# GStreamer/gst-plugins-rs

Measured on AMD Instinct MI355X. Metric: 4K RGBA frames/sec through hsvfilter+colorlut at 1 GPU; % HBM roofline, higher is better.
Workload: dtype u8

## Files before the change

gst-plugins-rs_amd/csrc/group.hip:

```cpp
#include "internal.hpp"

#include <chrono>
#include <condition_variable>
#include <algorithm>
#include <cstring>
#include <deque>
#include <mutex>
#include <unordered_map>
#include <vector>

using namespace mi355;

namespace {

struct Desc {
  mi355_ctx *ctx;
  uint8_t *src, *dst;
  int width, height, stride, format;
  mi355_hsv_settings hs;
  const uint32_t *table;
  std::shared_ptr<void> table_ref;
  bool batchable;
  bool fused;
  uint64_t ticket;
  hipEvent_t ready;
};

struct Batch {
  uint64_t seq;
  std::vector<uint64_t> tickets;
  hipEvent_t done;
  int waiters;
  std::shared_ptr<void> table_ref;
};

struct GroupCore {
  int device = 0;
  std::mutex mu;
  std::vector<hipEvent_t> events;
  uint64_t next_ticket = 1;
  std::string last_error;
};

hipEvent_t take_event(GroupCore *g) {
  if (!g->events.empty()) { hipEvent_t e = g->events.back(); g->events.pop_back(); return e; }
  hipEvent_t e = nullptr;
  if (hipEventCreateWithFlags(&e, hipEventDisableTiming) != hipSuccess) { (void)hipGetLastError(); return nullptr; }
  return e;
}

int fail(GroupCore *g, int status, const std::string &msg) {
  g->last_error = msg;
  return status;
}

int record_ready(GroupCore *g, mi355_ctx *ctx, hipEvent_t *ready) {
  *ready = nullptr;
  if (hipStreamQuery(ctx->stream) == hipSuccess) return MI355_OK;
  (void)hipGetLastError();
  hipEvent_t e = take_event(g);
  if (!e || hipEventRecord(e, ctx->stream) != hipSuccess) {
    (void)hipGetLastError();
    if (e) g->events.push_back(e);
    return fail(g, MI355_ERR_HIP, "group: hipEventRecord(ready)");
  }
  *ready = e;
  return MI355_OK;
}

enum class Waited { kNothing , kDone, kFailed };
template <class S>
Waited wait_seq_unlocking(std::deque<S> &sets, uint64_t seq, std::unique_lock<std::mutex> &lk) {
  S *mine = nullptr;
  for (S &s : sets)
    if (s.seq == seq) { mine = &s; break; }
  if (!mine) return Waited::kNothing;
  const hipEvent_t ev = mine->done;
  mine->waiters++;
  lk.unlock();
  const hipError_t e = hipEventSynchronize(ev);
  lk.lock();
  for (S &s : sets)
    if (s.seq == seq) { s.waiters--; break; }
  if (e != hipSuccess) { (void)hipGetLastError(); return Waited::kFailed; }
  return Waited::kDone;
}

// ... 622 lines not shown
        const auto deadline = std::chrono::steady_clock::now() + std::chrono::microseconds(linger_us);
        while (is_pending(ticket) && (int)pending.size() < expected) {
          if (cv.wait_until(lk, deadline) == std::cv_status::timeout) break;
        }
      }
      if (is_pending(ticket)) (void)flush_locked(g, ticket);
    }
    if (int rc = wait_unlocking(g, lk, ticket)) return rc;
    auto r = results.find(ticket);
    if (r == results.end()) return fail(g, MI355_ERR_INVALID_ARG, std::string("group: this ") + Kind::kItem + "'s result has been collected already");
    *out = std::move(r->second);
    results.erase(r);
    if (const int status = Kind::status(*out)) return fail(g, status, std::string("group: the launch that carried this ") + Kind::kItem + " failed");
    return MI355_OK;
  }

  void stats(uint64_t out[4]) const {
    out[0] = n_items;
    out[1] = n_sets;
    out[2] = n_largest;
    out[3] = n_launches;
  }

  void destroy(GroupCore *g) {
    if (!kind.lane_stream(0)) return;
    if (kind.set_up()) {
      std::lock_guard<std::mutex> lk(g->mu);
      (void)flush_locked(g);
    }
    for (int l = 0; l < kind.lanes(); l++) (void)hipStreamSynchronize(kind.lane_stream(l));
    for (Set &s : sets) {
      (void)hipEventDestroy(s.done);
      kind.blocks.give(&s.data.block);
    }
    sets.clear();
    for (Item &d : pending)
      if (d.ready) (void)hipEventDestroy(d.ready);
    pending.clear();
    kind.destroy();
  }
};

}

struct mi355_group : GroupCore {
  int max_batch = 8;
  hipStream_t stream = nullptr;
  std::vector<Desc> pending;
  std::deque<Batch> batches;
  std::unordered_map<uint64_t, uint64_t> where;
  std::unordered_map<uint64_t, int> failed;
  uint64_t next_seq = 1;
  uint64_t n_frames = 0, n_batched_launch_pairs = 0, n_single = 0;
  std::vector<std::shared_ptr<void>> dead_refs;
  SetQueue<CmpKind> cmp;
  SetQueue<CdKind> cd;
  SetQueue<HdKind> hd;
  SetQueue<YdKind> yd;
  SetQueue<HnKind> hn;
  SetQueue<HfKind> hf;
};

namespace {

struct Locked {
  std::vector<std::shared_ptr<void>> reap;
  mi355_group *g;
  std::unique_lock<std::mutex> lk;
  explicit Locked(mi355_group *g_) : g(g_), lk(g_->mu) {}
  ~Locked() {
    if (!lk.owns_lock()) lk.lock();
    reap.swap(g->dead_refs);
    lk.unlock();
  }
};

void retire_front(mi355_group *g) {
  Batch &b = g->batches.front();
  for (uint64_t t : b.tickets) g->where.erase(t);
  g->events.push_back(b.done);
  if (b.table_ref) g->dead_refs.push_back(std::move(b.table_ref));
  g->batches.pop_front();
}

void retire_done(mi355_group *g) {
  while (!g->batches.empty() && g->batches.front().waiters == 0) {
    if (hipEventQuery(g->batches.front().done) != hipSuccess) { (void)hipGetLastError(); break; }
    retire_front(g);
  }
}

bool same_class(const Desc &a, const Desc &b) {
  return a.batchable && b.batchable && a.fused == b.fused && a.width == b.width && a.height == b.height && a.stride == b.stride && a.format == b.format && a.table == b.table &&
         std::memcmp(&a.hs, &b.hs, sizeof(a.hs)) == 0 && a.ctx->force_generic == b.ctx->force_generic;
}

int flush_locked(mi355_group *g, uint64_t until = 0) {
  bool reached = false;
  while (!g->pending.empty() && !reached) {
    std::vector<Desc> take, keep;
    std::vector<mi355_ctx *> blocked;
    const Desc first = g->pending.front();
    for (const Desc &d : g->pending) {
      bool stream_blocked = false;
      for (mi355_ctx *c : blocked) stream_blocked |= c == d.ctx;
      const bool fits = take.empty() || (!stream_blocked && (int)take.size() < g->max_batch && same_class(first, d));
      if (fits) take.push_back(d);
      else keep.push_back(d);
      if (!stream_blocked) blocked.push_back(d.ctx);
    }
    g->pending.swap(keep);
    PixFmt fmt;
    (void)pixfmt_of(first.format, &fmt);
    hipEvent_t done = take_event(g);
    if (!done) return fail(g, MI355_ERR_HIP, "hipEventCreate");
    int rc = MI355_OK;
    if (first.batchable) {
      uint8_t *srcs[kMultiFrames], *dsts[kMultiFrames];
      for (size_t i = 0; i < take.size(); i++) {
        srcs[i] = take[i].src;
        dsts[i] = take[i].dst;
        if (take[i].ready && hipStreamWaitEvent(g->stream, take[i].ready, 0) != hipSuccess) rc = MI355_ERR_HIP;
      }
      if (!rc && !first.fused) rc = launch_hsvfilter_multi(first.ctx, g->stream, srcs, (int)take.size(), first.width, first.height, fmt, first.hs);
      if (!rc) rc = launch_colorlut_multi(first.ctx, g->stream, first.table, srcs, dsts, (int)take.size(), first.width, first.height, first.fused);
      if (!rc && hipEventRecord(done, g->stream) != hipSuccess) rc = MI355_ERR_HIP;
      g->n_batched_launch_pairs++;
    } else {
      const Desc &d = take[0];
      const size_t pitch = (size_t)d.stride * (size_t)d.height;
      if (!g->batches.empty() && hipStreamWaitEvent(d.ctx->stream, g->batches.back().done, 0) != hipSuccess) rc = MI355_ERR_HIP;
      if (!rc && d.fused) rc = launch_hsv_colorlut(d.ctx, d.src, pitch, d.stride, d.dst, pitch, d.stride, 1, d.width, d.height, d.hs);
      if (!rc && !d.fused) rc = launch_hsvfilter(d.ctx, d.src, 1, pitch, d.width, d.height, d.stride, fmt, d.hs);
      if (!rc && !d.fused) rc = launch_colorlut(d.ctx, d.src, pitch, d.stride, d.dst, pitch, d.stride, 1, d.width, d.height, d.format);
      if (!rc && hipEventRecord(done, d.ctx->stream) != hipSuccess) rc = MI355_ERR_HIP;
      if (!rc && hipStreamWaitEvent(g->stream, done, 0) != hipSuccess) rc = MI355_ERR_HIP;
      if (rc && rc != MI355_ERR_HIP) g->last_error = d.ctx->last_error;
      g->n_single++;
    }
    for (const Desc &d : take)
      if (d.ready) g->events.push_back(d.ready);
    if (rc) {
      (void)hipGetLastError();
      g->events.push_back(done);
      if (g->failed.size() > 65536) g->failed.clear();
      for (const Desc &d : take) g->failed[d.ticket] = rc;
      if (g->last_error.empty()) g->last_error = "group launch failed";
      return rc;
    }
    Batch b{g->next_seq++, {}, done, 0, first.batchable ? first.table_ref : std::shared_ptr<void>()};
    for (const Desc &d : take) { b.tickets.push_back(d.ticket); g->where[d.ticket] = b.seq; reached |= until != 0 && d.ticket == until; }
    g->batches.push_back(std::move(b));
    g->n_frames += take.size();
  }
  return MI355_OK;
}

int wait_unlocking(mi355_group *g, std::unique_lock<std::mutex> &lk, uint64_t ticket) {
  auto bad = g->failed.find(ticket);
  if (bad != g->failed.end()) {
    const int rc = bad->second;
    g->failed.erase(bad);
    return fail(g, rc, "group: the launch that carried this frame failed");
  }
  auto it = g->where.find(ticket);
  if (it == g->where.end()) return MI355_OK;
  const uint64_t seq = it->second;
  const Waited w = wait_seq_unlocking(g->batches, seq, lk);
  if (w == Waited::kNothing) return MI355_OK;
  if (w == Waited::kFailed) return fail(g, MI355_ERR_HIP, "hipEventSynchronize(group batch)");
  while (!g->batches.empty() && g->batches.front().seq <= seq && g->batches.front().waiters == 0) retire_front(g);
  return MI355_OK;
}

int wait_all_unlocking(mi355_group *g, std::unique_lock<std::mutex> &lk) {
  while (!g->batches.empty()) {
    const uint64_t t = g->batches.back().tickets.back();
    const size_t before = g->batches.size();
    int rc = wait_unlocking(g, lk, t);
    if (rc) return rc;
    if (!g->batches.empty() && g->batches.size() >= before && g->batches.back().tickets.back() == t) break;
  }
  return MI355_OK;
}


template <class F>
void for_each_queue_but_compare(mi355_group *g, F &&f) {
  f(g->cd);
  f(g->hd);
  f(g->yd);
  f(g->hn);
  f(g->hf);
}

template <class F>
void for_each_set_queue(mi355_group *g, F &&f) {
  f(g->cmp);
  for_each_queue_but_compare(g, f);
}

int refuse_set_queue_ticket(mi355_group *g, uint64_t ticket) {
  std::string owner;
  for_each_queue_but_compare(g, [&](auto &q) {
    if (owner.empty() && q.owns(ticket)) owner = q.foreign_refusal();
  });
  return owner.empty() ? MI355_OK : fail(g, MI355_ERR_INVALID_ARG, owner);
}


template <class Q>
int queue_set_rendezvous(mi355_group *g, Q mi355_group::*q, int expected_streams, unsigned linger_us) {
  if (!g || expected_streams < 0) return MI355_ERR_INVALID_ARG;
  Locked L(g);
  (g->*q).set_rendezvous(expected_streams, linger_us);
  return MI355_OK;
}

template <class Q>
int queue_stats(mi355_group *g, Q mi355_group::*q, uint64_t *stats, int columns = 4) {
  if (!g || !stats) return MI355_ERR_INVALID_ARG;
  std::lock_guard<std::mutex> lk(g->mu);
  uint64_t all[4];
  (g->*q).stats(all);
  std::copy(all, all + columns, stats);
  return MI355_OK;
}

template <class Q>
int queue_wait_status(mi355_group *g, Q mi355_group::*q, uint64_t ticket) {
  if (!g) return MI355_ERR_INVALID_ARG;
  Locked L(g);
  int status = MI355_OK;
  return (g->*q).wait(g, L.lk, ticket, &status);
}

}

extern "C" {

mi355_group *mi355_group_create(int device, int max_batch, int *status) {
  if (max_batch < 0 || max_batch > kMultiFrames) { if (status) *status = MI355_ERR_INVALID_ARG; return nullptr; }
  if (hipSetDevice(device) != hipSuccess) { (void)hipGetLastError(); if (status) *status = MI355_ERR_NO_DEVICE; return nullptr; }
  mi355_group *g = new mi355_group();
  g->device = device;
  g->max_batch = max_batch ? max_batch : 8;
  if (hipStreamCreateWithFlags(&g->stream, hipStreamNonBlocking) != hipSuccess) {
    (void)hipGetLastError();
    delete g;
    if (status) *status = MI355_ERR_HIP;
    return nullptr;
  }
  if (status) *status = MI355_OK;
  return g;
}

void mi355_group_destroy(mi355_group *g) {
  if (!g) return;
  (void)hipSetDevice(g->device);
  {
    Locked L(g);
    (void)flush_locked(g);
    (void)wait_all_unlocking(g, L.lk);
  }
  (void)hipStreamSynchronize(g->stream);
  for_each_set_queue(g, [&](auto &q) { q.destroy(g); });
  for (Batch &b : g->batches) (void)hipEventDestroy(b.done);
  for (Desc &d : g->pending)
    if (d.ready) (void)hipEventDestroy(d.ready);
  g->pending.clear();
  g->batches.clear();
  g->dead_refs.clear();
  for (hipEvent_t e : g->events) (void)hipEventDestroy(e);
  (void)hipStreamDestroy(g->stream);
  delete g;
}

const char *mi355_group_last_error(mi355_group *g) { return g ? g->last_error.c_str() : "null group"; }

static int submit_frame(mi355_group *g, mi355_ctx *ctx, uint8_t *d_src, uint8_t *d_dst, int width, int height, int stride, int format,
                        const mi355_hsv_settings *settings, uint64_t *ticket, bool fused) {
  if (!g) return MI355_ERR_INVALID_ARG;
  Locked L(g);
  PixFmt fmt;
  if (!ctx || !d_src || !d_dst || !settings || width <= 0 || height <= 0 || !pixfmt_of(format, &fmt) || (size_t)stride < (size_t)width * fmt.pixel_stride)
    return fail(g, MI355_ERR_INVALID_ARG, "group: bad frame");
  if (format != MI355_FMT_RGBA) return fail(g, MI355_ERR_INVALID_ARG, "group: hsvfilter ! colorlut takes RGBA frames only");
  if (ctx->device != g->device) return fail(g, MI355_ERR_INVALID_ARG, "group: context of another device");
  if (!ctx->lut.loaded) return fail(g, MI355_ERR_NOT_CONFIGURED, "No LUT configured");
  if (hipSetDevice(g->device) != hipSuccess) { (void)hipGetLastError(); return fail(g, MI355_ERR_HIP, "hipSetDevice"); }
  Desc d{};
  d.ctx = ctx; d.src = d_src; d.dst = d_dst; d.width = width; d.height = height; d.stride = stride; d.format = format; d.hs = *settings;
  d.fused = fused;
  retire_done(g);
  bool settled = true;
  if (fused) {
    if (std::memcmp(&ctx->group_fused_hs, settings, sizeof(*settings)) == 0) { if (ctx->group_fused_stable < 1000000u) ctx->group_fused_stable++; }
    else { ctx->group_fused_hs = *settings; ctx->group_fused_stable = 1; }
    settled = ctx->group_fused_stable >= 8u;
  }
  const uint8_t *one[1] = {d_src};
  d.batchable = settled && format == MI355_FMT_RGBA && (fused || d_src != d_dst) && hsvfilter_multi_applicable(one, 1, width, height, stride, fmt) && width % 4 == 0 &&
                width >= 128 && (uintptr_t)d_dst % 16 == 0 && ctx->lut_variant == 0 && ctx->hsv_table_mode != 2 && (!fused || ctx->lut.is3d);
  if (d.batchable && (fused ? colorlut_multi_fused_table(ctx, settings, &d.table) : colorlut_multi_table(ctx, &d.table)) != MI355_OK) {
    (void)hipGetLastError();
    d.batchable = false;
    d.table = nullptr;
  }
  if (d.batchable) d.table_ref = ctx->lut.table_ref[fused ? 1 : 0];
  if (int rc = record_ready(g, ctx, &d.ready)) return rc;
  d.ticket = g->next_ticket++;
  if (ticket) *ticket = d.ticket;
  g->pending.push_back(d);
  if ((int)g->pending.size() >= g->max_batch) (void)flush_locked(g, g->pending.front().ticket);
  return MI355_OK;
}

int mi355_group_submit_chain(mi355_group *g, mi355_ctx *ctx, uint8_t *d_src, uint8_t *d_dst, int width, int height, int stride, int format,
                             const mi355_hsv_settings *settings, uint64_t *ticket) {
  return submit_frame(g, ctx, d_src, d_dst, width, height, stride, format, settings, ticket, false);
}

int mi355_group_submit_fused(mi355_group *g, mi355_ctx *ctx, uint8_t *d_src, uint8_t *d_dst, int width, int height, int stride, int format,
                             const mi355_hsv_settings *settings, uint64_t *ticket) {
  return submit_frame(g, ctx, d_src, d_dst, width, height, stride, format, settings, ticket, true);
}

int mi355_group_flush(mi355_group *g) {
  if (!g) return MI355_ERR_INVALID_ARG;
  Locked L(g);
  if (hipSetDevice(g->device) != hipSuccess) { (void)hipGetLastError(); return fail(g, MI355_ERR_HIP, "hipSetDevice"); }
  int first = flush_locked(g);
  for_each_set_queue(g, [&](auto &q) {
    const int r = q.kind.set_up() ? q.flush_locked(g) : MI355_OK;
    if (!first) first = r;
  });
  return first;
}


int mi355_group_set_rendezvous(mi355_group *g, int expected_streams, unsigned linger_us) {
  return queue_set_rendezvous(g, &mi355_group::cmp, expected_streams, linger_us);
}

int mi355_group_set_compare_lanes(mi355_group *g, int lanes) {
  if (!g || lanes < 1 || lanes > kCmpMaxLanes) return MI355_ERR_INVALID_ARG;
  Locked L(g);
// ... 334 lines not shown
  bool is_pending = false;
  for (const Desc &d : g->pending) is_pending |= d.ticket == ticket;
  if (is_pending) {
    int rc = flush_locked(g, ticket);
    if (rc) return rc;
  }
  auto bad = g->failed.find(ticket);
  if (bad != g->failed.end()) return fail(g, bad->second, "group: the launch that carried this frame failed");
  auto it = g->where.find(ticket);
  if (it == g->where.end()) return MI355_OK;
  for (Batch &b : g->batches)
    if (b.seq == it->second) {
      if (hipStreamWaitEvent(ctx->stream, b.done, 0) != hipSuccess) { (void)hipGetLastError(); return fail(g, MI355_ERR_HIP, "hipStreamWaitEvent(group batch)"); }
      break;
    }
  return MI355_OK;
}

int mi355_group_wait_all(mi355_group *g) {
  if (!g) return MI355_ERR_INVALID_ARG;
  Locked L(g);
  std::unique_lock<std::mutex> &lk = L.lk;
  if (hipSetDevice(g->device) != hipSuccess) { (void)hipGetLastError(); return fail(g, MI355_ERR_HIP, "hipSetDevice"); }
  int rc = flush_locked(g);
  if (rc) return rc;
  if ((rc = wait_all_unlocking(g, lk))) return rc;
  for_each_queue_but_compare(g, [&](auto &q) {
    if (rc || !q.kind.set_up()) return;
    if (!(rc = q.flush_locked(g))) rc = q.wait_all_unlocking(g, lk);
  });
  return rc;
}

int mi355_group_submit_round(mi355_group *g, mi355_ctx *const *ctxs, int n_streams, uint8_t *const *d_src, uint8_t *const *d_dst, int width, int height,
                             int stride, int format, const mi355_hsv_settings *settings) {
  if (!g || !ctxs || !d_src || !d_dst || n_streams < 0) return MI355_ERR_INVALID_ARG;
  for (int i = 0; i < n_streams; i++) {
    int rc = mi355_group_submit_chain(g, ctxs[i], d_src[i], d_dst[i], width, height, stride, format, settings, nullptr);
    if (rc) return rc;
  }
  return mi355_group_flush(g);
}

int mi355_group_submit_round_fused(mi355_group *g, mi355_ctx *const *ctxs, int n_streams, uint8_t *const *d_src, uint8_t *const *d_dst, int width,
                                   int height, int stride, int format, const mi355_hsv_settings *settings) {
  if (!g || !ctxs || !d_src || !d_dst || n_streams < 0) return MI355_ERR_INVALID_ARG;
  for (int i = 0; i < n_streams; i++) {
    int rc = mi355_group_submit_fused(g, ctxs[i], d_src[i], d_dst[i], width, height, stride, format, settings, nullptr);
    if (rc) return rc;
  }
  return mi355_group_flush(g);
}

int mi355_group_stats(mi355_group *g, uint64_t stats[3]) {
  if (!g || !stats) return MI355_ERR_INVALID_ARG;
  std::lock_guard<std::mutex> lk(g->mu);
  stats[0] = g->n_frames;
  stats[1] = g->n_batched_launch_pairs;
  stats[2] = g->n_single;
  return MI355_OK;
}

}

namespace {
std::mutex g_pg_mu;
struct ProcessGroup { int device; mi355_group *g; int refs; };
std::vector<ProcessGroup> g_pg;
}

extern "C" {

mi355_group *mi355_group_shared(int device, int *status) {
  std::lock_guard<std::mutex> lk(g_pg_mu);
  for (ProcessGroup &p : g_pg)
    if (p.device == device) { p.refs++; if (status) *status = MI355_OK; return p.g; }
  mi355_group *g = mi355_group_create(device, 0, status);
  if (g) g_pg.push_back(ProcessGroup{device, g, 1});
  return g;
}

void mi355_group_release(mi355_group *g) {
  if (!g) return;
  bool last = false;
  {
    std::lock_guard<std::mutex> lk(g_pg_mu);
    for (size_t i = 0; i < g_pg.size(); i++)
      if (g_pg[i].g == g) {
        last = --g_pg[i].refs == 0;
        if (last) g_pg.erase(g_pg.begin() + (std::ptrdiff_t)i);
        break;
      }
  }
  if (last) mi355_group_destroy(g);
}

}
```

gst-plugins-rs_amd/mi355fx/__init__.py:

```python
import ctypes as C
import os

import numpy as np

_HERE = os.path.dirname(os.path.abspath(__file__))
PKG_ROOT = os.path.dirname(_HERE)
LIB_PATH = os.environ.get("MI355FX_LIB") or os.path.join(PKG_ROOT, "libmi355fx.so")
HEADER_PATH = os.path.join(os.path.dirname(PKG_ROOT), "include", "mi355fx.h")

FMT = {"RGBx": 0, "xRGB": 1, "BGRx": 2, "xBGR": 3, "RGBA": 4, "ARGB": 5, "BGRA": 6, "ABGR": 7,
       "RGB": 8, "BGR": 9, "RGBA64_LE": 10, "RGBA64_BE": 11}
FMT_LAYOUT = {"RGBx": (4, 0, 0), "RGBA": (4, 0, 0), "RGB": (3, 0, 0), "xRGB": (4, 1, 0), "ARGB": (4, 1, 0),
              "BGRx": (4, 0, 1), "BGRA": (4, 0, 1), "BGR": (3, 0, 1), "xBGR": (4, 1, 1), "ABGR": (4, 1, 1)}

OK, ERR_INVALID_ARG, ERR_NO_DEVICE, ERR_HIP, ERR_NOT_CONFIGURED, ERR_OOM, ERR_UNSUPPORTED, ERR_TIMEOUT = 0, -1, -2, -3, -4, -5, -6, -7
FLAG_FORCE_GENERIC = 1
FLAG_HSV_BLOCKS_PER_CU = 2
FLAG_FUSED_VARIANT = 3
FLAG_LUT_VARIANT = 4
FLAG_LUT_STAGGER = 5
FLAG_HSV_TABLE = 6
FLAG_BRICK_TILES_PER_RUN = 7
FLAG_BRICK_SETS = 8
FLAG_BRICK_PRIO = 9
# ... 253 lines not shown
        "mi355_ebur128_add_frames_batch_device": (i, [vp, vp, sz, i]),
        "mi355_ebur128_loudness_batch": (i, [vp, i, C.POINTER(C.c_double)]),
        "mi355_ebur128_peak_batch": (i, [vp, i, C.POINTER(C.c_double)]),
        "mi355_ebur128_reset": (i, [vp]),
        "mi355_ebur128_teardown": (i, [vp]),
        "mi355_ebur128_add_frames": (i, [vp, vp, sz, i]),
        "mi355_ebur128_add_frames_planar": (i, [vp, C.POINTER(vp), sz, i]),
        "mi355_ebur128_loudness_momentary": (i, [vp, C.POINTER(C.c_double)]),
        "mi355_ebur128_loudness_shortterm": (i, [vp, C.POINTER(C.c_double)]),
        "mi355_ebur128_loudness_global": (i, [vp, C.POINTER(C.c_double)]),
        "mi355_ebur128_relative_threshold": (i, [vp, C.POINTER(C.c_double)]),
        "mi355_ebur128_loudness_range": (i, [vp, C.POINTER(C.c_double)]),
        "mi355_ebur128_sample_peak": (i, [vp, C.c_uint, C.POINTER(C.c_double)]),
        "mi355_ebur128_true_peak": (i, [vp, C.c_uint, C.POINTER(C.c_double)]),
        "mi355_loudnorm_setup": (i, [vp, C.c_uint, C.c_double, C.c_double, C.c_double, C.c_double]),
        "mi355_loudnorm_push": (i, [vp, vp, sz, vp, sz, C.POINTER(sz)]),
        "mi355_loudnorm_drain": (i, [vp, vp, sz, C.POINTER(sz), C.POINTER(i)]),
        "mi355_loudnorm_teardown": (i, [vp]),
        "mi355_loudnorm_setup_batch": (i, [vp, C.c_uint, C.c_uint, C.c_double, C.c_double, C.c_double, C.c_double]),
        "mi355_loudnorm_batch_frame_size": (sz, [vp]),
        "mi355_loudnorm_process_batch": (i, [vp, vp, sz, sz, vp, sz, sz, C.POINTER(sz), i, i]),
        "mi355_host_alloc": (vp, [vp, sz]),
        "mi355_host_free": (i, [vp, vp]),
        "mi355_pipe_create": (vp, [vp, i, sz]),
        "mi355_pipe_destroy": (None, [vp]),
        "mi355_pipe_submit_hsvfilter": (i, [vp, u8p, sz, i, i, i, C.POINTER(HsvSettings), C.POINTER(C.c_uint64)]),
        "mi355_pipe_submit_colorlut": (i, [vp, u8p, i, u8p, i, i, i, i, C.POINTER(C.c_uint64)]),
        "mi355_pipe_submit_hsv_colorlut": (i, [vp, u8p, i, u8p, i, i, i, C.POINTER(HsvSettings), C.POINTER(C.c_uint64)]),
        "mi355_pipe_wait": (i, [vp, C.c_uint64]),
        "mi355_pipe_wait_all": (i, [vp]),
        "mi355_videocompare_hash_frame": (i, [vp, u8p, i, i, i, i, i, C.POINTER(C.c_uint64)]),
        "mi355_videocompare_hash_frames_device": (i, [vp, u8p, sz, i, i, i, i, i, i, C.POINTER(C.c_uint64)]),
        "mi355_videocompare_distance": (C.c_double, [i, C.c_uint64, C.c_uint64]),
        "mi355_dssim_create_image": (i, [vp, u8p, i, i, i, i, C.POINTER(vp)]),
        "mi355_dssim_create_image_device": (i, [vp, u8p, i, i, i, i, C.POINTER(vp)]),
        "mi355_dssim_free_image": (None, [vp, vp]),
        "mi355_dssim_compare": (i, [vp, vp, vp, C.POINTER(C.c_double)]),
        "mi355_dssim_compare_frames": (i, [vp, vp, C.POINTER(vp), i, i, i, i, i, C.POINTER(C.c_double)]),
        "mi355_dssim_compare_frames_device": (i, [vp, vp, C.POINTER(vp), i, i, i, i, i, C.POINTER(C.c_double)]),
        "mi355_issue_streams_round": (i, [C.POINTER(vp), i, C.POINTER(vp), C.POINTER(vp), i, i, i, i, C.POINTER(HsvSettings)]),
        "mi355_group_create": (vp, [i, i, C.POINTER(C.c_int)]),
        "mi355_group_destroy": (None, [vp]),
        "mi355_group_last_error": (C.c_char_p, [vp]),
        "mi355_group_submit_chain": (i, [vp, vp, u8p, u8p, i, i, i, i, C.POINTER(HsvSettings), C.POINTER(C.c_uint64)]),
        "mi355_group_submit_fused": (i, [vp, vp, u8p, u8p, i, i, i, i, C.POINTER(HsvSettings), C.POINTER(C.c_uint64)]),
        "mi355_group_flush": (i, [vp]),
        "mi355_pipe_set_group": (i, [vp, vp]),
        "mi355_group_wait": (i, [vp, C.c_uint64]),
        "mi355_group_order_after": (i, [vp, vp, C.c_uint64]),
        "mi355_group_wait_all": (i, [vp]),
        "mi355_group_stats": (i, [vp, C.POINTER(C.c_uint64)]),
        "mi355_group_set_rendezvous": (i, [vp, i, C.c_uint]),
        "mi355_group_set_compare_lanes": (i, [vp, i]),
        "mi355_group_submit_compare": (i, [vp, vp, u8p, u8p, i, i, i, i, i, C.POINTER(C.c_uint64)]),
        "mi355_group_wait_compare": (i, [vp, C.c_uint64, C.POINTER(C.c_double), C.POINTER(C.c_uint64)]),
        "mi355_group_compare_stats": (i, [vp, C.POINTER(C.c_uint64)]),
        "mi355_group_set_colordetect_rendezvous": (i, [vp, i, C.c_uint]),
        "mi355_group_submit_colordetect": (i, [vp, vp, vp, sz, i, i, i, C.POINTER(C.c_uint64)]),
        "mi355_group_wait_colordetect": (i, [vp, C.c_uint64, u8p, C.POINTER(C.c_int)]),
        "mi355_group_colordetect_stats": (i, [vp, C.POINTER(C.c_uint64)]),
        "mi355_selftest_colordetect_plan": (i, [i, i, C.POINTER(C.c_uint64), C.POINTER(C.c_uint32), C.POINTER(C.c_uint32), C.POINTER(C.c_uint64),
                                                C.POINTER(C.c_uint32)]),
        "mi355_group_set_hsvdetect_rendezvous": (i, [vp, i, C.c_uint]),
        "mi355_group_submit_hsvdetect": (i, [vp, vp, u8p, i, i, u8p, i, i, i, i, C.POINTER(HsvDetectSettings), C.POINTER(C.c_uint64)]),
        "mi355_group_wait_hsvdetect": (i, [vp, C.c_uint64]),
        "mi355_group_hsvdetect_stats": (i, [vp, C.POINTER(C.c_uint64)]),
        "mi355_selftest_hsvdetect_plan": (i, [i, i, C.c_uint, i, C.POINTER(C.c_uint64), C.POINTER(C.c_uint32), C.POINTER(C.c_uint32),
                                              C.POINTER(C.c_uint32)]),
        "mi355_group_set_hsvfilter_rendezvous": (i, [vp, i, C.c_uint]),
        "mi355_group_submit_hsvfilter": (i, [vp, vp, u8p, i, i, i, i, C.POINTER(HsvSettings), C.POINTER(C.c_uint64)]),
        "mi355_group_wait_hsvfilter": (i, [vp, C.c_uint64]),
        "mi355_group_hsvfilter_stats": (i, [vp, C.POINTER(C.c_uint64)]),
        "mi355_selftest_hsvfilter_set_plan": (i, [i, C.POINTER(HsvFilterPlanFrame), i, C.POINTER(HsvFilterPlanOut), C.POINTER(C.c_int)]),
        "mi355_agroup_create_echo": (vp, [i, i, sz, C.POINTER(C.c_int)]),
        "mi355_agroup_create_ebur128": (vp, [i, i, C.c_uint, C.c_uint, C.c_uint, C.POINTER(C.c_int), C.POINTER(C.c_int)]),
        "mi355_agroup_create_loudnorm": (vp, [i, i, C.c_uint, C.c_double, C.c_double, C.c_double, C.c_double, C.POINTER(C.c_int)]),
        "mi355_agroup_destroy": (None, [vp]),
        "mi355_agroup_last_error": (C.c_char_p, [vp]),
        "mi355_agroup_set_linger": (i, [vp, C.c_uint, C.c_uint]),
        "mi355_agroup_detach": (i, [vp, i]),
        "mi355_agroup_submit_echo": (i, [vp, i, vp, sz, i, sz, C.c_double, C.c_double, i, C.POINTER(C.c_uint64)]),
        "mi355_agroup_submit_ebur128": (i, [vp, i, vp, sz, i, i, C.POINTER(C.c_uint64)]),
        "mi355_agroup_ebur128_reset": (i, [vp, i]),
        "mi355_agroup_submit_loudnorm": (i, [vp, i, vp, sz, vp, sz, i, i, C.POINTER(C.c_uint64)]),
        "mi355_agroup_loudnorm_frame_size": (sz, [vp, i]),
        "mi355_agroup_wait": (i, [vp, C.c_uint64, C.POINTER(sz)]),
        "mi355_agroup_ebur128_loudness": (i, [vp, i, i, C.POINTER(C.c_double)]),
        "mi355_agroup_ebur128_peak": (i, [vp, i, i, C.c_uint, C.POINTER(C.c_double)]),
        "mi355_agroup_echo_get_state": (i, [vp, i, vp, sz, C.POINTER(sz)]),
        "mi355_agroup_stats": (i, [vp, C.POINTER(C.c_uint64)]),
        "mi355_agroup_loudnorm_push": (i, [vp, i, vp, sz, vp, sz, C.POINTER(sz)]),
        "mi355_agroup_loudnorm_drain": (i, [vp, i, vp, sz, C.POINTER(sz), C.POINTER(C.c_int)]),
        "mi355_agroup_shared_echo": (vp, [i, i, sz, C.POINTER(C.c_int), C.POINTER(C.c_int)]),
        "mi355_agingradio_setup": (i, [vp, C.c_uint, C.c_uint, C.c_uint, C.c_uint64]),
        "mi355_agingradio_process": (i, [vp, vp, sz, i, C.POINTER(AgingRadioSettings)]),
        "mi355_agingradio_process_device": (i, [vp, vp, sz, i, C.POINTER(AgingRadioSettings)]),
        "mi355_agingradio_get_state": (i, [vp, C.POINTER(C.c_double), C.c_uint, C.POINTER(C.c_uint64)]),
        "mi355_agingradio_reset": (i, [vp]),
        "mi355_agroup_create_agingradio": (vp, [i, i, C.POINTER(C.c_int)]),
        "mi355_agroup_shared_agingradio": (vp, [i, i, C.POINTER(C.c_int), C.POINTER(C.c_int)]),
        "mi355_agroup_agingradio_setup": (i, [vp, i, C.c_uint, C.c_uint, C.c_uint, C.c_uint64]),
        "mi355_agroup_submit_agingradio": (i, [vp, i, vp, sz, i, C.POINTER(AgingRadioSettings), i, C.POINTER(C.c_uint64)]),
        "mi355_agroup_agingradio_get_state": (i, [vp, i, C.POINTER(C.c_double), C.c_uint, C.POINTER(C.c_uint64)]),
        "mi355_mixer_setup": (i, [vp, C.c_uint, C.c_uint, vp]),
        "mi355_mixer_setup_minus1": (i, [vp, C.c_uint]),
        "mi355_mixer_process": (i, [vp, C.POINTER(MixerSegment), C.c_uint, C.POINTER(MixerOutput), C.c_uint, sz]),
# ... 204 lines not shown
    def __init__(self, device=0, max_batch=0):
        self.L = load_library()
        st = C.c_int(0)
        self.h = self.L.mi355_group_create(device, max_batch, C.byref(st))
        if not self.h:
            raise Mi355Error(st.value, "mi355_group_create")
        self._rounds = {}
        self._yolodec_caps = {}
        self._handdec_landmarks = set()

    def _ck(self, rc):
        if rc != 0:
            raise Mi355Error(rc, (self.L.mi355_group_last_error(self.h) or b"").decode())

    def submit_chain(self, ctx, d_src, d_dst, width, height, stride, fmt, settings):
        s = HsvSettings(*[float(v) for v in settings])
        t = C.c_uint64(0)
        self._ck(self.L.mi355_group_submit_chain(self.h, ctx.h, d_src, d_dst, width, height, stride, FMT[fmt], C.byref(s), C.byref(t)))
        return t.value

    def submit_fused(self, ctx, d_src, d_dst, width, height, stride, fmt, settings):
        s = HsvSettings(*[float(v) for v in settings])
        t = C.c_uint64(0)
        self._ck(self.L.mi355_group_submit_fused(self.h, ctx.h, d_src, d_dst, width, height, stride, FMT[fmt], C.byref(s), C.byref(t)))
        return t.value

    def submit_round(self, contexts, src_ptrs, dst_ptrs, width, height, stride, fmt, settings, fused=False):
        key = (tuple(c.h for c in contexts), tuple(src_ptrs), tuple(dst_ptrs))
        arr = self._rounds.get(key)
        if arr is None:
            n = len(contexts)
            arr = self._rounds[key] = ((C.c_void_p * n)(*[c.h for c in contexts]), (C.c_void_p * n)(*src_ptrs), (C.c_void_p * n)(*dst_ptrs))
        hs = HsvSettings(*[float(v) for v in settings])
        fn = self.L.mi355_group_submit_round_fused if fused else self.L.mi355_group_submit_round
        self._ck(fn(self.h, arr[0], len(contexts), arr[1], arr[2], width, height, stride, FMT[fmt], C.byref(hs)))

    def flush(self):
        self._ck(self.L.mi355_group_flush(self.h))

    def wait(self, ticket):
        self._ck(self.L.mi355_group_wait(self.h, ticket))

    def order_after(self, ctx, ticket):
        self._ck(self.L.mi355_group_order_after(self.h, ctx.h, ticket))

    def wait_all(self):
        self._ck(self.L.mi355_group_wait_all(self.h))

    def stats(self):
        c = (C.c_uint64 * 3)()
        self._ck(self.L.mi355_group_stats(self.h, c))
        return int(c[0]), int(c[1]), int(c[2])

    def set_rendezvous(self, expected_streams, linger_us):
        self._ck(self.L.mi355_group_set_rendezvous(self.h, expected_streams, linger_us))

    def set_compare_lanes(self, lanes):
        self._ck(self.L.mi355_group_set_compare_lanes(self.h, lanes))

    def submit_compare(self, ctx, d_ref, d_frame, stride, width, height, fmt="RGBA", algo=5):
        t = C.c_uint64(0)
        self._ck(self.L.mi355_group_submit_compare(self.h, ctx.h, d_ref, d_frame, stride, width, height, FMT[fmt], algo, C.byref(t)))
        return t.value

    def wait_compare(self, ticket):
        d = C.c_double(0.0)
        h = (C.c_uint64 * 2)()
        self._ck(self.L.mi355_group_wait_compare(self.h, ticket, C.byref(d), h))
        return d.value, int(h[0]), int(h[1])

    def compare_stats(self):
        c = (C.c_uint64 * 3)()
        self._ck(self.L.mi355_group_compare_stats(self.h, c))
        return int(c[0]), int(c[1]), int(c[2])

    def set_colordetect_rendezvous(self, expected_streams, linger_us):
        self._ck(self.L.mi355_group_set_colordetect_rendezvous(self.h, expected_streams, linger_us))

    def submit_colordetect(self, ctx, d_data, data_len, fmt, quality=10, max_colors=2):
        t = C.c_uint64(0)
        self._ck(self.L.mi355_group_submit_colordetect(self.h, ctx.h, d_data, data_len, FMT[fmt], quality, max_colors, C.byref(t)))
        return t.value

    def wait_colordetect(self, ticket):
        pal = np.zeros(255 * 3, np.uint8)
        n = C.c_int(0)
        self._ck(self.L.mi355_group_wait_colordetect(self.h, ticket, pal.ctypes.data, C.byref(n)))
        return [tuple(int(v) for v in pal[3 * k: 3 * k + 3]) for k in range(n.value)]

    def colordetect_stats(self):
        c = (C.c_uint64 * 4)()
        self._ck(self.L.mi355_group_colordetect_stats(self.h, c))
        return int(c[0]), int(c[1]), int(c[2]), int(c[3])

    def set_hsvdetect_rendezvous(self, expected_streams, linger_us):
        self._ck(self.L.mi355_group_set_hsvdetect_rendezvous(self.h, expected_streams, linger_us))

    def submit_hsvdetect(self, ctx, d_src, src_stride, src_fmt, d_dst, dst_stride, dst_fmt, width, height, settings):
        s = None if settings is None else C.byref(HsvDetectSettings(*[float(v) for v in settings]))
        t = C.c_uint64(0)
        self._ck(self.L.mi355_group_submit_hsvdetect(self.h, ctx.h, d_src, src_stride, FMT[src_fmt], d_dst, dst_stride, FMT[dst_fmt], width, height, s,
                                                     C.byref(t)))
        return t.value

    def wait_hsvdetect(self, ticket):
        self._ck(self.L.mi355_group_wait_hsvdetect(self.h, ticket))
# ... 1369 lines not shown
```

include/mi355fx.h:

```cpp
#ifndef MI355FX_H
#define MI355FX_H

#include <stddef.h>
#include <stdint.h>

#ifdef __cplusplus
extern "C" {
#endif

#define MI355FX_ABI_VERSION 1

typedef enum mi355_status {
  MI355_OK = 0,
  MI355_ERR_INVALID_ARG = -1,
  MI355_ERR_NO_DEVICE = -2,
  MI355_ERR_HIP = -3,
  MI355_ERR_NOT_CONFIGURED = -4,
  MI355_ERR_OUT_OF_MEMORY = -5,
  MI355_ERR_UNSUPPORTED = -6,
  MI355_ERR_TIMEOUT = -7
} mi355_status;

typedef enum mi355_video_format {
  MI355_FMT_RGBX = 0,
// ... 62 lines not shown
                             int format, const mi355_hsv_settings *settings);
int mi355_hsvfilter_frames_device(mi355_ctx *ctx, uint8_t *d_data, int n_frames, size_t frame_pitch,
                                  int width, int height, int stride, int format,
                                  const mi355_hsv_settings *settings);

typedef struct mi355_hsvdetect_settings {
  float hue_ref, hue_var;
  float saturation_ref, saturation_var;
  float value_ref, value_var;
} mi355_hsvdetect_settings;

int mi355_hsvdetect_frame(mi355_ctx *ctx, const uint8_t *src, size_t src_len, int src_stride,
                          int src_format, uint8_t *dst, size_t dst_len, int dst_stride,
                          int dst_format, int width, const mi355_hsvdetect_settings *settings);
int mi355_hsvdetect_frames_device(mi355_ctx *ctx, const uint8_t *d_src, size_t src_pitch,
                                  int src_stride, int src_format, uint8_t *d_dst, size_t dst_pitch,
                                  int dst_stride, int dst_format, int n_frames, int width,
                                  int height, const mi355_hsvdetect_settings *settings);

int mi355_colorlut_load(mi355_ctx *ctx, int is3d, size_t size, const float *table,
                        const float domain_scale[3], const float domain_offset[3]);
int mi355_colorlut_unload(mi355_ctx *ctx);
int mi355_colorlut_kernel_choice(mi355_ctx *ctx, int fused, int *table_in_use, double *ms_per_mpx_compute, double *ms_per_mpx_table);
int mi355_shared_table_count(void);
const char *mi355_colorlut_last_kernel(mi355_ctx *ctx);
int mi355_colorlut_brick_stats(mi355_ctx *ctx, uint64_t counters[2], double *last_miss_fraction, int *level, int reset);
int mi355_colorlut_window_stats(mi355_ctx *ctx, uint64_t counters[3], int reset);
int mi355_selftest_brickwatch(int n_calls, const double *miss0, const double *slow0, const double *miss1, const double *slow1, int lag,
                              int *level_out);
int mi355_selftest_autopick(int n_calls, const uint64_t *n_vec, const double *ms_compute, const double *ms_table, int lag,
                            int *kind_out, int *measured_out);
int mi355_colorlut_frame(mi355_ctx *ctx, const uint8_t *src, int src_stride, uint8_t *dst,
                         int dst_stride, int width, int height, int format);
int mi355_colorlut_frames_device(mi355_ctx *ctx, const uint8_t *d_src, size_t src_pitch,
                                 int src_stride, uint8_t *d_dst, size_t dst_pitch, int dst_stride,
                                 int n_frames, int width, int height, int format);

int mi355_issue_streams_round(mi355_ctx *const *ctxs, int n_streams, uint8_t *const *d_src, uint8_t *const *d_dst,
                              int width, int height, int stride, int format, const mi355_hsv_settings *settings);

typedef struct mi355_group mi355_group;
mi355_group *mi355_group_create(int device, int max_batch, int *status);
void mi355_group_destroy(mi355_group *group);
const char *mi355_group_last_error(mi355_group *group);
int mi355_group_submit_chain(mi355_group *group, mi355_ctx *ctx, uint8_t *d_src, uint8_t *d_dst, int width, int height,
                             int stride, int format, const mi355_hsv_settings *settings, uint64_t *ticket);
int mi355_group_submit_fused(mi355_group *group, mi355_ctx *ctx, uint8_t *d_src, uint8_t *d_dst, int width, int height,
                             int stride, int format, const mi355_hsv_settings *settings, uint64_t *ticket);
int mi355_group_flush(mi355_group *group);
int mi355_group_order_after(mi355_group *group, mi355_ctx *ctx, uint64_t ticket);
int mi355_group_wait(mi355_group *group, uint64_t ticket);
int mi355_group_wait_all(mi355_group *group);
int mi355_group_stats(mi355_group *group, uint64_t stats[3]);
int mi355_group_submit_round(mi355_group *group, mi355_ctx *const *ctxs, int n_streams, uint8_t *const *d_src,
                             uint8_t *const *d_dst, int width, int height, int stride, int format,
                             const mi355_hsv_settings *settings);
int mi355_group_submit_round_fused(mi355_group *group, mi355_ctx *const *ctxs, int n_streams, uint8_t *const *d_src,
                                   uint8_t *const *d_dst, int width, int height, int stride, int format,
                                   const mi355_hsv_settings *settings);

int mi355_group_set_rendezvous(mi355_group *group, int expected_streams, unsigned linger_us);
int mi355_group_set_compare_lanes(mi355_group *group, int lanes);
int mi355_group_submit_compare(mi355_group *group, mi355_ctx *ctx, const uint8_t *d_ref, const uint8_t *d_frame, int stride, int width, int height,
                               int format, int algo, uint64_t *ticket);
int mi355_group_wait_compare(mi355_group *group, uint64_t ticket, double *distance, uint64_t hashes[2]);
int mi355_group_compare_stats(mi355_group *group, uint64_t stats[3]);

#define MI355_COLORDETECT_SET_MAX 32
int mi355_group_set_colordetect_rendezvous(mi355_group *group, int expected_streams, unsigned linger_us);
int mi355_group_submit_colordetect(mi355_group *group, mi355_ctx *ctx, const uint8_t *d_data, size_t data_len, int format, int quality,
                                   int max_colors, uint64_t *ticket);
int mi355_group_wait_colordetect(mi355_group *group, uint64_t ticket, uint8_t palette_rgb[255 * 3], int *n_colors);
int mi355_group_colordetect_stats(mi355_group *group, uint64_t stats[4]);
int mi355_selftest_colordetect_plan(int n_cu, int n_jobs, const uint64_t *n_samples, uint32_t *first_block, uint32_t *blocks,
                                    uint64_t *samples_per_block, uint32_t *total_blocks);

#define MI355_HSVDETECT_SET_MAX 32
int mi355_group_set_hsvdetect_rendezvous(mi355_group *group, int expected_streams, unsigned linger_us);
int mi355_group_submit_hsvdetect(mi355_group *group, mi355_ctx *ctx, const uint8_t *d_src, int src_stride, int src_format,
                                 uint8_t *d_dst, int dst_stride, int dst_format, int width, int height,
                                 const mi355_hsvdetect_settings *settings, uint64_t *ticket);
int mi355_group_wait_hsvdetect(mi355_group *group, uint64_t ticket);
int mi355_group_hsvdetect_stats(mi355_group *group, uint64_t stats[4]);
int mi355_selftest_hsvdetect_plan(int n_cu, int blocks_per_cu, unsigned units_per_block, int n_jobs, const uint64_t *units,
                                  uint32_t *first_block, uint32_t *blocks, uint32_t *total_blocks);

#define MI355_HSVFILTER_SET_MAX 32
typedef struct mi355_hsvfilter_plan_frame {
  uint64_t address;
  int32_t width, height, stride, format;
  mi355_hsv_settings settings;
  int32_t force_generic;
} mi355_hsvfilter_plan_frame;
typedef struct mi355_hsvfilter_plan_out {
  int32_t set, launch, variant;
  uint32_t first_block, blocks, reserved;
  uint64_t units;
} mi355_hsvfilter_plan_out;
int mi355_group_set_hsvfilter_rendezvous(mi355_group *group, int expected_streams, unsigned linger_us);
int mi355_group_submit_hsvfilter(mi355_group *group, mi355_ctx *ctx, uint8_t *d_data, int width, int height, int stride,
                                 int format, const mi355_hsv_settings *settings, uint64_t *ticket);
int mi355_group_wait_hsvfilter(mi355_group *group, uint64_t ticket);
int mi355_group_hsvfilter_stats(mi355_group *group, uint64_t stats[4]);
int mi355_selftest_hsvfilter_set_plan(int n_cu, const mi355_hsvfilter_plan_frame *frames, int n_frames,
                                      mi355_hsvfilter_plan_out *out, int *n_sets);

// ... 463 lines not shown
```

Before: 44470.

## Spread fused group batches across multiple lane streams with hazard-tracked dependencies

Fused batchable group launches now go round-robin across up to four non-blocking lane streams instead of the single group stream. A LanePlan tracks the live batches and adds cross-stream event waits only when a new batch's src/dst ranges overlap an earlier one on another stream, or the two share a context. Retire and wait-all logic now handle batches finishing out of order per stream. The aim is to let independent fused batches overlap on the GPU, at the cost of extra bookkeeping on the host, more streams, and O(n) searches through the live batches.

```diff
diff --git a/gst-plugins-rs_amd/csrc/group.hip b/gst-plugins-rs_amd/csrc/group.hip
--- a/gst-plugins-rs_amd/csrc/group.hip
+++ b/gst-plugins-rs_amd/csrc/group.hip
@@ -1,4 +1,5 @@
 #include "internal.hpp"
+#include "lanes.hpp"
 
 #include <chrono>
 #include <condition_variable>
@@ -28,11 +29,14 @@
 
 struct Batch {
   uint64_t seq;
+  hipStream_t stream;
   std::vector<uint64_t> tickets;
   hipEvent_t done;
   int waiters;
   std::shared_ptr<void> table_ref;
 };
+
+constexpr int kFusedLanesDefault = 4;
 
 struct GroupCore {
   int device = 0;
@@ -761,6 +765,11 @@
   std::unordered_map<uint64_t, int> failed;
   uint64_t next_seq = 1;
   uint64_t n_frames = 0, n_batched_launch_pairs = 0, n_single = 0;
+  int n_lanes = kFusedLanesDefault;
+  bool lanes_made = false;
+  hipStream_t lanes[kFusedLanesMax] = {};
+  LanePlan plan;
+  uint64_t lane_batches[kFusedLanesMax] = {}, lane_waits = 0, lane_no_wait = 0;
   std::vector<std::shared_ptr<void>> dead_refs;
   SetQueue<CmpKind> cmp;
   SetQueue<CdKind> cd;
@@ -784,18 +793,29 @@
   }
 };
 
-void retire_front(mi355_group *g) {
-  Batch &b = g->batches.front();
+void retire_at(mi355_group *g, size_t i) {
+  Batch &b = g->batches[i];
   for (uint64_t t : b.tickets) g->where.erase(t);
   g->events.push_back(b.done);
   if (b.table_ref) g->dead_refs.push_back(std::move(b.table_ref));
-  g->batches.pop_front();
-}
-
-void retire_done(mi355_group *g) {
-  while (!g->batches.empty() && g->batches.front().waiters == 0) {
-    if (hipEventQuery(g->batches.front().done) != hipSuccess) { (void)hipGetLastError(); break; }
-    retire_front(g);
+  g->plan.finished(b.seq);
+  g->batches.erase(g->batches.begin() + (std::ptrdiff_t)i);
+}
+
+void retire_done(mi355_group *g, bool front_only = false) {
+  hipStream_t busy[kFusedLanesMax + 1];
+  size_t n_busy = 0;
+  const size_t n_streams = front_only || !g->lanes_made || g->n_lanes == 1 ? 1 : (size_t)g->n_lanes + 1;
+  for (size_t i = 0; i < g->batches.size() && n_busy < n_streams;) {
+    Batch &b = g->batches[i];
+    bool skip = false;
+    for (size_t k = 0; k < n_busy; k++) skip |= busy[k] == b.stream;
+    if (!skip && b.waiters == 0 && hipEventQuery(b.done) == hipSuccess) { retire_at(g, i); continue; }
+    if (!skip) {
+      if (b.waiters == 0) (void)hipGetLastError();
+      busy[n_busy++] = b.stream;
+    }
+    i++;
   }
 }
 
@@ -824,21 +844,55 @@
     hipEvent_t done = take_event(g);
     if (!done) return fail(g, MI355_ERR_HIP, "hipEventCreate");
     int rc = MI355_OK;
+    hipStream_t stream = g->stream;
+    if (g->n_lanes > 1) retire_done(g);
+    LaneBatch use{g->next_seq, (uintptr_t)g->stream, {}};
+    for (const Desc &d : take) use.frames.push_back(LaneFrame{d.ctx, (uintptr_t)d.src, (uintptr_t)d.dst, (size_t)d.stride * (size_t)d.height, !d.fused});
     if (first.batchable) {
+      if (first.fused) {
+        if (!g->lanes_made) {
+          for (int l = 0; l < g->n_lanes && g->n_lanes > 1 && !rc; l++)
+            if (hipStreamCreateWithFlags(&g->lanes[l], hipStreamNonBlocking) != hipSuccess) rc = MI355_ERR_HIP;
+          g->lanes_made = true;
+        }
+        const int lane = g->n_lanes > 1 ? g->plan.next_lane(g->n_lanes) : 0;
+        if (g->n_lanes > 1) stream = g->lanes[lane];
+        if (!stream) rc = MI355_ERR_HIP;
+        g->lane_batches[lane]++;
+      }
+      if (g->n_lanes > 1 && !rc) {
+        use.stream = (uintptr_t)stream;
+        std::vector<uint64_t> deps;
+        g->plan.depends_on(use, &deps);
+        for (uint64_t seq : deps)
+          for (const Batch &b : g->batches)
+            if (b.seq == seq && hipStreamWaitEvent(stream, b.done, 0) != hipSuccess) rc = MI355_ERR_HIP;
+        g->lane_waits += deps.size();
+        if (deps.empty()) g->lane_no_wait++;
+      } else if (!rc) g->lane_no_wait++;
       uint8_t *srcs[kMultiFrames], *dsts[kMultiFrames];
       for (size_t i = 0; i < take.size(); i++) {
         srcs[i] = take[i].src;
         dsts[i] = take[i].dst;
-        if (take[i].ready && hipStreamWaitEvent(g->stream, take[i].ready, 0) != hipSuccess) rc = MI355_ERR_HIP;
+        if (!rc && take[i].ready && hipStreamWaitEvent(stream, take[i].ready, 0) != hipSuccess) rc = MI355_ERR_HIP;
       }
-      if (!rc && !first.fused) rc = launch_hsvfilter_multi(first.ctx, g->stream, srcs, (int)take.size(), first.width, first.height, fmt, first.hs);
-      if (!rc) rc = launch_colorlut_multi(first.ctx, g->stream, first.table, srcs, dsts, (int)take.size(), first.width, first.height, first.fused);
-      if (!rc && hipEventRecord(done, g->stream) != hipSuccess) rc = MI355_ERR_HIP;
+      if (!rc && !first.fused) rc = launch_hsvfilter_multi(first.ctx, stream, srcs, (int)take.size(), first.width, first.height, fmt, first.hs);
+      if (!rc) rc = launch_colorlut_multi(first.ctx, stream, first.table, srcs, dsts, (int)take.size(), first.width, first.height, first.fused);
+      if (!rc && hipEventRecord(done, stream) != hipSuccess) rc = MI355_ERR_HIP;
       g->n_batched_launch_pairs++;
     } else {
       const Desc &d = take[0];
       const size_t pitch = (size_t)d.stride * (size_t)d.height;
-      if (!g->batches.empty() && hipStreamWaitEvent(d.ctx->stream, g->batches.back().done, 0) != hipSuccess) rc = MI355_ERR_HIP;
+      hipStream_t seen[kFusedLanesMax + 1];
+      size_t n_seen = 0;
+      for (size_t i = g->batches.size(); i-- > 0 && n_seen < sizeof(seen) / sizeof(seen[0]);) {
+        const Batch &b = g->batches[i];
+        bool later_one = false;
+        for (size_t k = 0; k < n_seen; k++) later_one |= seen[k] == b.stream;
+        if (later_one) continue;
+        seen[n_seen++] = b.stream;
+        if (hipStreamWaitEvent(d.ctx->stream, b.done, 0) != hipSuccess) rc = MI355_ERR_HIP;
+      }
       if (!rc && d.fused) rc = launch_hsv_colorlut(d.ctx, d.src, pitch, d.stride, d.dst, pitch, d.stride, 1, d.width, d.height, d.hs);
       if (!rc && !d.fused) rc = launch_hsvfilter(d.ctx, d.src, 1, pitch, d.width, d.height, d.stride, fmt, d.hs);
       if (!rc && !d.fused) rc = launch_colorlut(d.ctx, d.src, pitch, d.stride, d.dst, pitch, d.stride, 1, d.width, d.height, d.format);
@@ -857,9 +911,10 @@
       if (g->last_error.empty()) g->last_error = "group launch failed";
       return rc;
     }
-    Batch b{g->next_seq++, {}, done, 0, first.batchable ? first.table_ref : std::shared_ptr<void>()};
+    Batch b{g->next_seq++, first.batchable ? stream : g->stream, {}, done, 0, first.batchable ? first.table_ref : std::shared_ptr<void>()};
     for (const Desc &d : take) { b.tickets.push_back(d.ticket); g->where[d.ticket] = b.seq; reached |= until != 0 && d.ticket == until; }
     g->batches.push_back(std::move(b));
+    g->plan.launched(std::move(use));
     g->n_frames += take.size();
   }
   return MI355_OK;
@@ -878,18 +933,24 @@
   const Waited w = wait_seq_unlocking(g->batches, seq, lk);
   if (w == Waited::kNothing) return MI355_OK;
   if (w == Waited::kFailed) return fail(g, MI355_ERR_HIP, "hipEventSynchronize(group batch)");
-  while (!g->batches.empty() && g->batches.front().seq <= seq && g->batches.front().waiters == 0) retire_front(g);
+  retire_done(g);
   return MI355_OK;
 }
 
 int wait_all_unlocking(mi355_group *g, std::unique_lock<std::mutex> &lk) {
-  while (!g->batches.empty()) {
-    const uint64_t t = g->batches.back().tickets.back();
-    const size_t before = g->batches.size();
-    int rc = wait_unlocking(g, lk, t);
-    if (rc) return rc;
-    if (!g->batches.empty() && g->batches.size() >= before && g->batches.back().tickets.back() == t) break;
-  }
+  std::vector<uint64_t> last;
+  hipStream_t seen[kFusedLanesMax + 1];
+  size_t n_seen = 0;
+  for (size_t i = g->batches.size(); i-- > 0 && n_seen < sizeof(seen) / sizeof(seen[0]);) {
+    const Batch &b = g->batches[i];
+    bool later_one = false;
+    for (size_t k = 0; k < n_seen; k++) later_one |= seen[k] == b.stream;
+    if (later_one) continue;
+    seen[n_seen++] = b.stream;
+    last.push_back(b.tickets.back());
+  }
+  for (uint64_t t : last)
+    if (int rc = wait_unlocking(g, lk, t)) return rc;
   return MI355_OK;
 }
 
@@ -973,6 +1034,8 @@
     (void)wait_all_unlocking(g, L.lk);
   }
   (void)hipStreamSynchronize(g->stream);
+  for (hipStream_t lane : g->lanes)
+    if (lane) (void)hipStreamSynchronize(lane);
   for_each_set_queue(g, [&](auto &q) { q.destroy(g); });
   for (Batch &b : g->batches) (void)hipEventDestroy(b.done);
   for (Desc &d : g->pending)
@@ -982,6 +1045,8 @@
   g->dead_refs.clear();
   for (hipEvent_t e : g->events) (void)hipEventDestroy(e);
   (void)hipStreamDestroy(g->stream);
+  for (hipStream_t lane : g->lanes)
+    if (lane) (void)hipStreamDestroy(lane);
   delete g;
 }
 
@@ -1001,7 +1066,7 @@
   Desc d{};
   d.ctx = ctx; d.src = d_src; d.dst = d_dst; d.width = width; d.height = height; d.stride = stride; d.format = format; d.hs = *settings;
   d.fused = fused;
-  retire_done(g);
+  retire_done(g, true);
   bool settled = true;
   if (fused) {
     if (std::memcmp(&ctx->group_fused_hs, settings, sizeof(*settings)) == 0) { if (ctx->group_fused_stable < 1000000u) ctx->group_fused_stable++; }
@@ -1442,6 +1507,23 @@
   return mi355_group_flush(g);
 }
 
+int mi355_group_set_fused_lanes(mi355_group *g, int lanes) {
+  if (!g || lanes < 1 || lanes > kFusedLanesMax) return MI355_ERR_INVALID_ARG;
+  Locked L(g);
+  if (g->lanes_made) return fail(g, MI355_ERR_INVALID_ARG, "group: the fused lanes exist already (set them before the first fused batch)");
+  g->n_lanes = lanes;
+  return MI355_OK;
+}
+
+int mi355_group_fused_lane_stats(mi355_group *g, uint64_t stats[6]) {
+  if (!g || !stats) return MI355_ERR_INVALID_ARG;
+  std::lock_guard<std::mutex> lk(g->mu);
+  std::copy(g->lane_batches, g->lane_batches + kFusedLanesMax, stats);
+  stats[4] = g->lane_waits;
+  stats[5] = g->lane_no_wait;
+  return MI355_OK;
+}
+
 int mi355_group_stats(mi355_group *g, uint64_t stats[3]) {
   if (!g || !stats) return MI355_ERR_INVALID_ARG;
   std::lock_guard<std::mutex> lk(g->mu);
diff --git a/gst-plugins-rs_amd/csrc/lanes.hpp b/gst-plugins-rs_amd/csrc/lanes.hpp
--- /dev/null
+++ b/gst-plugins-rs_amd/csrc/lanes.hpp
@@ -0,0 +1,68 @@
+#pragma once
+#include <cstddef>
+#include <cstdint>
+#include <utility>
+#include <vector>
+
+namespace mi355 {
+
+constexpr int kFusedLanesMax = 4;
+
+struct LaneFrame {
+  const void *ctx;
+  uintptr_t src, dst;
+  size_t bytes;
+  bool src_written;
+};
+
+struct LaneBatch {
+  uint64_t seq;
+  uintptr_t stream;
+  std::vector<LaneFrame> frames;
+};
+
+inline bool lane_ranges_overlap(uintptr_t a, uintptr_t b, size_t bytes_a, size_t bytes_b) { return a < b + bytes_b && b < a + bytes_a; }
+
+inline bool lane_frames_ordered(const LaneFrame &earlier, const LaneFrame &later) {
+  if (earlier.ctx == later.ctx) return true;
+  const LaneFrame &e = earlier, &l = later;
+  if (lane_ranges_overlap(e.dst, l.src, e.bytes, l.bytes)) return true;
+  if (lane_ranges_overlap(e.dst, l.dst, e.bytes, l.bytes)) return true;
+  if (lane_ranges_overlap(e.src, l.dst, e.bytes, l.bytes)) return true;
+  return (e.src_written || l.src_written) && lane_ranges_overlap(e.src, l.src, e.bytes, l.bytes);
+}
+
+struct LanePlan {
+  std::vector<LaneBatch> live;
+  unsigned dealt = 0;
+
+  int next_lane(int n_lanes) { return (int)(dealt++ % (unsigned)(n_lanes < 1 ? 1 : n_lanes)); }
+
+  void depends_on(const LaneBatch &b, std::vector<uint64_t> *out) const {
+    out->clear();
+    uintptr_t answered[kFusedLanesMax + 2];
+    size_t n_answered = 0;
+    for (size_t i = live.size(); i-- > 0;) {
+      const LaneBatch &e = live[i];
+      if (e.stream == b.stream) continue;
+      bool skip = false;
+      for (size_t k = 0; k < n_answered; k++) skip |= answered[k] == e.stream;
+      if (skip) continue;
+      bool ordered = false;
+      for (size_t x = 0; x < e.frames.size() && !ordered; x++)
+        for (size_t y = 0; y < b.frames.size() && !ordered; y++) ordered = lane_frames_ordered(e.frames[x], b.frames[y]);
+      if (!ordered) continue;
+      out->push_back(e.seq);
+      if (n_answered < sizeof(answered) / sizeof(answered[0])) answered[n_answered++] = e.stream;
+    }
+  }
+
+  void launched(LaneBatch &&b) { live.push_back(std::move(b)); }
+
+  void finished(uint64_t seq) {
+    for (size_t i = 0; i < live.size(); i++)
+      if (live[i].seq == seq) { live.erase(live.begin() + (std::ptrdiff_t)i); return; }
+  }
+};
+
+}
diff --git a/gst-plugins-rs_amd/mi355fx/__init__.py b/gst-plugins-rs_amd/mi355fx/__init__.py
--- a/gst-plugins-rs_amd/mi355fx/__init__.py
+++ b/gst-plugins-rs_amd/mi355fx/__init__.py
@@ -329,6 +329,8 @@
         "mi355_group_stats": (i, [vp, C.POINTER(C.c_uint64)]),
         "mi355_group_set_rendezvous": (i, [vp, i, C.c_uint]),
         "mi355_group_set_compare_lanes": (i, [vp, i]),
+        "mi355_group_set_fused_lanes": (i, [vp, i]),
+        "mi355_group_fused_lane_stats": (i, [vp, C.POINTER(C.c_uint64)]),
         "mi355_group_submit_compare": (i, [vp, vp, u8p, u8p, i, i, i, i, i, C.POINTER(C.c_uint64)]),
         "mi355_group_wait_compare": (i, [vp, C.c_uint64, C.POINTER(C.c_double), C.POINTER(C.c_uint64)]),
         "mi355_group_compare_stats": (i, [vp, C.POINTER(C.c_uint64)]),
@@ -639,6 +641,14 @@
         self._ck(self.L.mi355_group_stats(self.h, c))
         return int(c[0]), int(c[1]), int(c[2])
 
+    def set_fused_lanes(self, lanes):
+        self._ck(self.L.mi355_group_set_fused_lanes(self.h, lanes))
+
+    def fused_lane_stats(self):
+        c = (C.c_uint64 * 6)()
+        self._ck(self.L.mi355_group_fused_lane_stats(self.h, c))
+        return tuple(int(v) for v in c[:4]), int(c[4]), int(c[5])
+
     def set_rendezvous(self, expected_streams, linger_us):
         self._ck(self.L.mi355_group_set_rendezvous(self.h, expected_streams, linger_us))
 
diff --git a/include/mi355fx.h b/include/mi355fx.h
--- a/include/mi355fx.h
+++ b/include/mi355fx.h
@@ -138,6 +138,8 @@
 int mi355_group_wait(mi355_group *group, uint64_t ticket);
 int mi355_group_wait_all(mi355_group *group);
 int mi355_group_stats(mi355_group *group, uint64_t stats[3]);
+int mi355_group_set_fused_lanes(mi355_group *group, int lanes);
+int mi355_group_fused_lane_stats(mi355_group *group, uint64_t stats[6]);
 int mi355_group_submit_round(mi355_group *group, mi355_ctx *const *ctxs, int n_streams, uint8_t *const *d_src,
                              uint8_t *const *d_dst, int width, int height, int stride, int format,
                              const mi355_hsv_settings *settings);
```

Result: no change. 44470 (median of 2 runs) (-0.0%).
